# AwsGeek/thinvids

Hardware: AMD Instinct MI355X
Metric: encoded frames/sec (whole node) at fixed PSNR, 1080p & 4K HEVC, 1/2/4/8 MI355X (higher is better)
Workload: dtype uint8 video / int32 integer transforms (bit-exact HEVC)

## Files before the change

### csrc/core/capi.cpp

```cpp
#include <cstring>
#include <exception>
#include <memory>
#include <string>
#include <vector>

#include "tv/av1_enc.h"
#include "tv/container.h"
#include "tv/cpu_encoder.h"
#include "tv/hevc_codec.h"
#include "tv/me_model.h"
#include "tv/sdh.h"
#include "tv/synth.h"
#include "tv/synth_tile.h"
#include "tv/tb_frag.h"

using namespace tv;

namespace {
thread_local std::string g_err;
template <class F> int guard(F&& f) {
  try {
    f();
    return 0;
  } catch (const std::exception& e) {
// ... 110 lines not shown
    uint8_t* P = c == 0 ? y : (c == 1 ? u : v);
    const int pw = c ? cw / 2 : cw, ph = c ? ch / 2 : ch;
    for (int y0 = 0; y0 < ph; y0 += tile_h)
      for (int x0 = 0; x0 < pw; x0 += tile_w)
        synth_tile_fill(ctx, c, x0, y0, tv_min(tile_w, pw - x0), tv_min(tile_h, ph - y0), pw, P);
  }
}

int tv_satd8x8(const int* d, int stride) { return satd8x8(d, stride); }

int tv_sao_picture_cpu(int W, int H, int qp, const uint8_t* sy, const uint8_t* su, const uint8_t* sv,
                       const uint8_t* dy, const uint8_t* du, const uint8_t* dv, uint32_t* params, uint8_t* oy,
                       uint8_t* ou, uint8_t* ov) {
  if (W <= 0 || H <= 0 || W % kCtb || H % kCtb || qp < 0 || qp > 51) {
    g_err = "tv_sao_picture_cpu: bad geometry or QP";
    return -1;
  }
  return guard([&] {
    Picture src, deb;
    src.alloc(W, H);
    deb.alloc(W, H);
    const uint8_t* s[3] = {sy, su, sv};
    const uint8_t* d[3] = {dy, du, dv};
    uint8_t* o[3] = {oy, ou, ov};
    for (int c = 0; c < 3; ++c) {
      const size_t n = (size_t)src.pw(c) * src.ph(c);
      std::memcpy(src.plane(c), s[c], n);
      std::memcpy(deb.plane(c), d[c], n);
    }
    sao_decide_picture(src, deb, qp, params);
    sao_picture(deb, params);
    for (int c = 0; c < 3; ++c) std::memcpy(o[c], deb.plane(c), (size_t)deb.pw(c) * deb.ph(c));
  });
}

void* tv_cpu_encoder_new(int width, int height, int qp, int deblock, int range, int max_merge) {
  SeqConfig cfg;
  cfg.width = width;
  cfg.height = height;
  cfg.qp = qp;
  cfg.set_flags(deblock);
  cfg.max_merge_cand = max_merge;
  cfg.finalize();
  CpuEncoder* e = nullptr;
  guard([&] { e = new CpuEncoder(cfg, range); });
  return e;
}
void* tv_cpu_encoder_new_b(int width, int height, int qp, int deblock, int range, int max_merge, int mgop) {
  SeqConfig cfg;
  cfg.width = width;
  cfg.height = height;
  cfg.qp = qp;
  cfg.set_flags(deblock);
  cfg.max_merge_cand = max_merge;
  cfg.mgop = mgop;
  cfg.finalize();
  CpuEncoder* e = nullptr;
  guard([&] { e = new CpuEncoder(cfg, range); });
  return e;
}
int tv_cpu_encoder_begin_gop(void* e, int nframes, int* disp) {
  return guard([&] {
    auto* enc = static_cast<CpuEncoder*>(e);
    enc->begin_gop(nframes);
    for (size_t k = 0; k < enc->plan().pics.size(); ++k) disp[k] = enc->plan().pics[k].disp;
  });
// ... 248 lines not shown
```

### csrc/gpu/k_frame.hip

```cpp
#include <cstring>

#include "gpu_common.h"
#include "k_encode.h"
#include "tv/synth.h"
#include "tv/synth_tile.h"

namespace tv {
namespace gpu {

constexpr int kSynTW = kSynthTileW, kSynTH = kSynthTileH, kSynRows = kSynTH / 4;
static_assert(kSynTW == 256 && kSynTH % 4 == 0, "a wave of 4-sample items spans the tile; 4 waves share its rows");

struct SynthArgs {
  SynthObject obj[kSynthObjects];
  int32_t t[kMaxBatch];
  int32_t ox[kMaxBatch][kSynthObjects], oy[kMaxBatch][kSynthObjects];
};
static_assert(sizeof(SynthArgs) + sizeof(Geo) + sizeof(FrameSet) + 16 <= 4096, "kernel arguments are limited to 4 KB");

constexpr int kSynSpanX = (kSynTW - 1) * 16, kSynSpanY = (kSynTH - 1) * 16;
constexpr int syn_max(int a, int b) { return a > b ? a : b; }
constexpr int syn_pts(int lp, int s) { return synth_win_max(kSynSpanX << s, lp) * synth_win_max(kSynSpanY << s, lp); }
constexpr int syn_rows(int lp, int s) { return synth_win_max(kSynSpanY << s, lp); }
constexpr int syn_lat_size(bool tex) {
// ... 161 lines not shown
  const int ntx = c ? ncx : nlx, ty = id / ntx, x0 = (id - ty * ntx) * kSynTW, y0 = ty * kSynTH;
  if (c)
    syn_tile<kTex, true>(top, lat, src, g, seed, a, c, x0, y0);
  else
    syn_tile<kTex, false>(top, lat, src, g, seed, a, 0, x0, y0);
}

__global__ void __launch_bounds__(256) k_sse(FrameSet a, FrameSet r, Geo g, unsigned long long* sse) {
  const int c = blockIdx.y, b = blockIdx.z;
  const int pw = c ? g.W / 2 : g.W;
  const int dw = c ? g.dw / 2 : g.dw, dh = c ? g.dh / 2 : g.dh;
  const uint8_t* A = a.plane(c, b, g);
  const uint8_t* R = r.plane(c, b, g);
  const int wq = (dw + 3) >> 2;
  unsigned s = 0;
  for (int i = blockIdx.x * blockDim.x + threadIdx.x; i < wq * dh; i += gridDim.x * blockDim.x) {
    const int y = i / wq, x = (i - y * wq) * 4;
    const uint32_t va = *reinterpret_cast<const uint32_t*>(A + (long)y * pw + x);
    const uint32_t vr = *reinterpret_cast<const uint32_t*>(R + (long)y * pw + x);
#pragma unroll
    for (int k = 0; k < 4; ++k) {
      const int d = (int)((va >> (8 * k)) & 255) - (int)((vr >> (8 * k)) & 255);
      s += (x + k < dw) ? (unsigned)(d * d) : 0u;
    }
  }
  unsigned long long t = s;
  for (int o = 32; o > 0; o >>= 1) t += __shfl_xor(t, o, 64);
  __shared__ unsigned long long part[4];
  if ((threadIdx.x & 63) == 0) part[threadIdx.x >> 6] = t;
  __syncthreads();
  if (threadIdx.x == 0) atomicAdd(sse + b * 3 + c, part[0] + part[1] + part[2] + part[3]);
}

typedef short tv_short2 __attribute__((ext_vector_type(2)));

__device__ constexpr uint32_t pack_taps4(int f, int k0) {
  return (uint32_t)(uint8_t)kLumaFilter[f][k0] | (uint32_t)(uint8_t)kLumaFilter[f][k0 + 1] << 8 |
         (uint32_t)(uint8_t)kLumaFilter[f][k0 + 2] << 16 | (uint32_t)(uint8_t)kLumaFilter[f][k0 + 3] << 24;
}
__device__ constexpr uint32_t pack_taps2(int f, int k0) {
  return (uint32_t)(uint16_t)kLumaFilter[f][k0] | (uint32_t)(uint16_t)kLumaFilter[f][k0 + 1] << 16;
}
__device__ __forceinline__ int dot4(uint32_t a, uint32_t b, int c) {
  return __builtin_amdgcn_sdot4((int)a, (int)b, c, false);
}
__device__ __forceinline__ int dot2(uint32_t a, uint32_t b, int c) {
  return __builtin_amdgcn_sdot2(__builtin_bit_cast(tv_short2, a), __builtin_bit_cast(tv_short2, b), c, false);
}
__device__ __forceinline__ uint32_t pack4_pixels(int v0, int v1, int v2, int v3) {
  return (uint32_t)clip_pixel(v0) | (uint32_t)clip_pixel(v1) << 8 | (uint32_t)clip_pixel(v2) << 16 |
         (uint32_t)clip_pixel(v3) << 24;
}

constexpr int kPhW = 10;
__global__ void __launch_bounds__(256) k_phase_planes(FrameSet ref, uint8_t* phase, Geo g) {
  const int tid = threadIdx.x;
  const int L = xcd_remap(blockIdx.x + gridDim.x * (blockIdx.y + gridDim.y * blockIdx.z),
                          gridDim.x * gridDim.y * gridDim.z);
  const int tpf = gridDim.x * gridDim.y, b = L / tpf, tyi = (L - b * tpf) / gridDim.x;
  const int tx0 = (L - b * tpf - tyi * gridDim.x) * 32 - 8, ty0 = tyi * 32 - 8;
  const uint8_t* R = ref.plane(0, b, g);
  __shared__ uint32_t raw[39][kPhW];
  __shared__ __align__(16) int16_t hf[3][39][32];
  for (int i = tid; i < 39 * kPhW; i += 256) {
    const int rr = i / kPhW, w = i - rr * kPhW;
    const uint8_t* row = R + (long)clip3(0, g.H - 1, ty0 - 3 + rr) * g.W;
    const int x = tx0 - 4 + 4 * w;
    uint32_t v;
    if (x >= 0 && x + 3 < g.W) {
      v = *reinterpret_cast<const uint32_t*>(row + x);
    } else {
      v = 0;
#pragma unroll
      for (int k = 0; k < 4; ++k) v |= (uint32_t)row[clip3(0, g.W - 1, x + k)] << (8 * k);
    }
    raw[rr][w] = v ^ 0x80808080u;
  }
  __syncthreads();
  for (int i = tid; i < 39 * 8; i += 256) {
    const int rr = i >> 3, c4 = i & 7;
    const uint32_t w0 = raw[rr][c4], w1 = raw[rr][c4 + 1], w2 = raw[rr][c4 + 2];
    int out[3][4];
#pragma unroll
    for (int j = 0; j < 4; ++j) {
      const uint32_t lo = j == 3 ? w1 : __builtin_amdgcn_alignbyte(w1, w0, j + 1);
      const uint32_t hi = j == 3 ? w2 : __builtin_amdgcn_alignbyte(w2, w1, j + 1);
#pragma unroll
      for (int f = 1; f < 4; ++f) out[f - 1][j] = dot4(lo, pack_taps4(f, 0), dot4(hi, pack_taps4(f, 4), 8192));
    }
#pragma unroll
    for (int f = 0; f < 3; ++f) {
      uint2 v;
      v.x = (uint32_t)(uint16_t)out[f][0] | (uint32_t)out[f][1] << 16;
      v.y = (uint32_t)(uint16_t)out[f][2] | (uint32_t)out[f][3] << 16;
      *reinterpret_cast<uint2*>(&hf[f][rr][4 * c4]) = v;
    }
  }
  __syncthreads();
  const int r = tid >> 3, c0 = (tid & 7) * 4;
  const int X = tx0 + c0, Y = ty0 + r;
  if (X + 8 >= g.pw16 || Y >= g.H + 8) return;
  uint8_t* base = phase + (long)b * 16 * g.psz + (long)(Y + 8) * g.pw16 + (X + 8);
  auto store = [&](int plane, uint32_t w) { *reinterpret_cast<uint32_t*>(base + (long)plane * g.psz) = w; };
  {
    uint32_t R8[8];
#pragma unroll
    for (int k = 0; k < 8; ++k) R8[k] = raw[r + k][(c0 >> 2) + 1];
    store(0, R8[3] ^ 0x80808080u);
    uint32_t C[2][4];
#pragma unroll
    for (int h = 0; h < 2; ++h) {
      const uint32_t* q = R8 + 4 * h;
      const uint32_t t01l = __builtin_amdgcn_perm(q[1], q[0], 0x05010400u);
      const uint32_t t01h = __builtin_amdgcn_perm(q[1], q[0], 0x07030602u);
      const uint32_t t23l = __builtin_amdgcn_perm(q[3], q[2], 0x05010400u);
      const uint32_t t23h = __builtin_amdgcn_perm(q[3], q[2], 0x07030602u);
      C[h][0] = __builtin_amdgcn_perm(t23l, t01l, 0x05040100u);
      C[h][1] = __builtin_amdgcn_perm(t23l, t01l, 0x07060302u);
      C[h][2] = __builtin_amdgcn_perm(t23h, t01h, 0x05040100u);
      C[h][3] = __builtin_amdgcn_perm(t23h, t01h, 0x07060302u);
    }
#pragma unroll
    for (int fy = 1; fy < 4; ++fy) {
      int v[4];
#pragma unroll
      for (int j = 0; j < 4; ++j)
        v[j] = dot4(C[0][j], pack_taps4(fy, 0), dot4(C[1][j], pack_taps4(fy, 4), 8192 + 32)) >> 6;
      store(4 * fy, pack4_pixels(v[0], v[1], v[2], v[3]));
    }
  }
#pragma unroll
  for (int fx = 1; fx < 4; ++fx) {
    uint2 H8[8];
#pragma unroll
    for (int k = 0; k < 8; ++k) H8[k] = *reinterpret_cast<const uint2*>(&hf[fx - 1][r + k][c0]);
    {
      const int h0 = (int16_t)(H8[3].x & 0xffff), h1 = (int16_t)(H8[3].x >> 16);
      const int h2 = (int16_t)(H8[3].y & 0xffff), h3 = (int16_t)(H8[3].y >> 16);
      store(fx, pack4_pixels((h0 + 32) >> 6, (h1 + 32) >> 6, (h2 + 32) >> 6, (h3 + 32) >> 6));
    }
    uint32_t P[4][4];
#pragma unroll
    for (int m = 0; m < 4; ++m) {
      P[m][0] = __builtin_amdgcn_perm(H8[2 * m + 1].x, H8[2 * m].x, 0x05040100u);
      P[m][1] = __builtin_amdgcn_perm(H8[2 * m + 1].x, H8[2 * m].x, 0x07060302u);
      P[m][2] = __builtin_amdgcn_perm(H8[2 * m + 1].y, H8[2 * m].y, 0x05040100u);
      P[m][3] = __builtin_amdgcn_perm(H8[2 * m + 1].y, H8[2 * m].y, 0x07060302u);
    }
#pragma unroll
    for (int fy = 1; fy < 4; ++fy) {
      int v[4];
#pragma unroll
      for (int j = 0; j < 4; ++j) {
        int a = dot2(P[0][j], pack_taps2(fy, 0), 0);
        a = dot2(P[1][j], pack_taps2(fy, 2), a);
        a = dot2(P[2][j], pack_taps2(fy, 4), a);
        a = dot2(P[3][j], pack_taps2(fy, 6), a);
        v[j] = ((a >> 6) + 32) >> 6;
      }
      store(fx + 4 * fy, pack4_pixels(v[0], v[1], v[2], v[3]));
    }
  }
}

__global__ void __launch_bounds__(256) __attribute__((amdgpu_waves_per_eu(8, 8))) k_deblock(FrameSet rec, DecisionSet dec, Geo g, int horizontal) {
  const int b = blockIdx.y;
  const int qp = dec.qp[b];
  const long ub = b * g.usz;
  const uint8_t* cl = dec.cu_log2 + ub;
  const uint8_t* in = dec.intra + ub;
  const uint8_t* cb = dec.cbf + ub;
  const int16_t* mv = dec.mv + 2 * ub;
  const uint8_t* dir = dec.dir ? dec.dir + ub : nullptr;
  const int16_t* mv1 = dec.mv1 ? dec.mv1 + 2 * ub : nullptr;
  const uint8_t* tu = dec.tu ? dec.tu + ub : nullptr;
  uint8_t* Y = rec.plane(0, b, g);
  uint8_t* U = rec.plane(1, b, g);
  uint8_t* V = rec.plane(2, b, g);
  const int W = g.W, H = g.H, Wc = W / 2;
  const int qpc = chroma_qp(qp, 0);
  const int nl = horizontal ? (H / 8 - 1) * (W / 4) : (W / 8 - 1) * (H / 4);
  const int nc = horizontal ? (H / 16 - 1) * (Wc / 4) : (W / 16 - 1) * (H / 8);
  auto ld = [](const uint8_t* p) { return *reinterpret_cast<const uint32_t*>(p); };
  auto st = [](uint8_t* p, uint32_t v) { *reinterpret_cast<uint32_t*>(p) = v; };
  for (int i = blockIdx.x * blockDim.x + threadIdx.x; i < nl + nc; i += gridDim.x * blockDim.x) {
    if (i < nl) {
      if (!horizontal) {
        const int x = 8 * (1 + i % (W / 8 - 1)), y = 4 * (i / (W / 8 - 1));
        const int bs = deblock_edge_bs(cl, in, cb, mv, g.w8, x - 1, y, x, y, dir, mv1, tu);
        if (bs) {
          uint32_t v[4][2];
#pragma unroll
          for (int k = 0; k < 4; ++k) {
// ... 87 lines not shown
    const int b = (int)(i / f16);
    const long r = i - b * f16;
    const uint4 v = reinterpret_cast<const uint4*>(frames + b * seg_stride)[r];
    uint4* d = r < y16 ? reinterpret_cast<uint4*>(src.y + b * g.ysz) + r
               : r < y16 + c16 ? reinterpret_cast<uint4*>(src.u + b * g.csz) + (r - y16)
                               : reinterpret_cast<uint4*>(src.v + b * g.csz) + (r - y16 - c16);
    *d = v;
  }
}
void launch_gather_frames(const uint8_t* frames, long seg_stride, FrameSet src, const Geo& g, int B, hipStream_t s) {
  const long n = B * (g.ysz + 2 * g.csz) / 16;
  k_gather_frames<<<(unsigned)tv_min(4096L, (n + 255) / 256), 256, 0, s>>>(frames, seg_stride, src, g, B);
}
struct QpArgs {
  int8_t q[64];
};
__global__ void __launch_bounds__(64) k_set_qp(int8_t* dst, QpArgs a, int n) {
  if ((int)threadIdx.x < n) dst[threadIdx.x] = a.q[threadIdx.x];
}
void launch_set_qp(int8_t* dst, const int8_t* host, int n, hipStream_t s) {
  for (int o = 0; o < n; o += 64) {
    QpArgs a;
    const int m = n - o < 64 ? n - o : 64;
    std::memcpy(a.q, host + o, (size_t)m);
    k_set_qp<<<1, 64, 0, s>>>(dst + o, a, m);
  }
}

void launch_sse(FrameSet a, FrameSet r, const Geo& g, unsigned long long* sse, int B, hipStream_t s) {
  dim3 grid((unsigned)tv_min(256, (int)((g.ysz / 4 + 4095) / 4096)), 3, B);
  k_sse<<<grid, 256, 0, s>>>(a, r, g, sse);
}
void launch_phase_planes(FrameSet ref, uint8_t* phase, const Geo& g, int B, hipStream_t s) {
  dim3 grid((g.W + 16 + 31) / 32, (g.H + 16 + 31) / 32, B);
  k_phase_planes<<<grid, 256, 0, s>>>(ref, phase, g);
}
constexpr int kSaoStrip = 4;
constexpr int kSaoRows = 34, kSaoRowsC = 18;
constexpr int kSaoPd = 16 * kSaoStrip + 2, kSaoPdC = 8 * kSaoStrip + 2;
constexpr int kSaoLumaDw = kSaoRows * kSaoPd, kSaoChromaDw = kSaoRowsC * kSaoPdC;
constexpr int kSaoTileDw = kSaoLumaDw + 2 * kSaoChromaDw;
constexpr int kSaoSrcDw = 8 * kSaoStrip + 2, kSaoSrcDwC = 4 * kSaoStrip + 2;
static_assert(kSaoSrcDw <= 64 && kSaoSrcDwC <= 32, "a tile row is staged by one wave (chroma: one half per plane)");
static_assert(8 * (kSaoTileDw * 4 + 64) <= 160 * 1024, "8 workgroups per CU");
typedef short sao_s2 __attribute__((ext_vector_type(2)));
__device__ __forceinline__ sao_s2 sao_pair(uint32_t w) { return __builtin_bit_cast(sao_s2, w); }
typedef unsigned short sao_u2 __attribute__((ext_vector_type(2)));
__device__ __forceinline__ sao_u2 sao_upair(sao_s2 w) { return __builtin_bit_cast(sao_u2, w); }
__device__ __forceinline__ sao_s2 sao_sign2(sao_s2 d) {
  const sao_s2 z = {0, 0};
  const sao_u2 f = {15, 15};
  return (d >> 15) | __builtin_bit_cast(sao_s2, __builtin_bit_cast(sao_u2, z - d) >> f);
}
__device__ __forceinline__ sao_s2 sao_relu2(sao_s2 e) { return e & ~(e >> 15); }
__device__ __forceinline__ sao_s2 sao_pkmax(sao_s2 a, sao_s2 b) {
  uint32_t r;
  asm("v_pk_max_i16 %0, %1, %2" : "=v"(r) : "v"(__builtin_bit_cast(uint32_t, a)), "v"(__builtin_bit_cast(uint32_t, b)));
  return sao_pair(r);
}
__device__ __forceinline__ sao_s2 sao_pkmin(sao_s2 a, sao_s2 b) {
  uint32_t r;
  asm("v_pk_min_i16 %0, %1, %2" : "=v"(r) : "v"(__builtin_bit_cast(uint32_t, a)), "v"(__builtin_bit_cast(uint32_t, b)));
  return sao_pair(r);
}
__device__ __forceinline__ sao_s2 sao_clamp1(sao_s2 d) {
  return sao_pkmin(sao_pkmax(d, sao_s2{-1, -1}), sao_s2{1, 1});
}
// ... 372 lines not shown
```

### csrc/gpu/k_stage.hip

```cpp
#include <hip/hip_runtime.h>

#include <string>

#include "gpu_common.h"
#include "k_encode.h"

namespace tv {
namespace gpu {

__global__ void __launch_bounds__(256) k_pad_plane(const uint8_t* __restrict__ src, int sw, int sh, int sstride, long sfs,
                                                   uint8_t* __restrict__ dst, int pw, int ph, int dstride, long dfs) {
  const int f = blockIdx.z, y = blockIdx.y;
  const int x0 = (blockIdx.x * 256 + threadIdx.x) * 4;
  if (x0 >= pw) return;
  const uint8_t* S = src + f * sfs + (long)tv_min(y, sh - 1) * sstride;
  uint8_t* D = dst + f * dfs + (long)y * dstride;
#pragma unroll
  for (int k = 0; k < 4; ++k)
    if (x0 + k < pw) D[x0 + k] = S[tv_min(x0 + k, sw - 1)];
}

template <typename T>
__global__ void __launch_bounds__(256) k_thumbs8(const T* __restrict__ y, int tw, int stride, long fs, float* out,
                                                 float scale) {
// ... 76 lines not shown
  for (int b = 0; b < B; ++b)
    if (qp[b] < 0 || qp[b] > 51) {
      g_stage_err = "tv_sao_batch: bad QP";
      return -1;
    }
  using namespace tv::gpu;
  hipStream_t st = static_cast<hipStream_t>(stream);
  const Geo g = make_geo(w, h);
  auto set = [&](const uint8_t* p) {
    uint8_t* q = const_cast<uint8_t*>(p);
    return FrameSet{q, q + B * g.ysz, q + B * g.ysz + B * g.csz};
  };
  RcTables t{};
  for (int q = 0; q < 52; ++q) t.sao_lam16[q] = tv::sao_lambda16(q);
  RcTables* rc = nullptr;
  int8_t* dqp = nullptr;
  bool ok = hipMalloc(&rc, sizeof(RcTables)) == hipSuccess && hipMalloc(&dqp, (size_t)B) == hipSuccess &&
            hipMemcpyAsync(rc, &t, sizeof(RcTables), hipMemcpyHostToDevice, st) == hipSuccess &&
            hipMemcpyAsync(dqp, qp, (size_t)B, hipMemcpyHostToDevice, st) == hipSuccess &&
            hipMemsetAsync(sse, 0, (size_t)B * 3 * sizeof(unsigned long long), st) == hipSuccess;
  if (ok) {
    launch_sao(set(src), set(deb), set(out), sao, dqp, rc, g, B, st, sse);
    ok = hipStreamSynchronize(st) == hipSuccess;
  }
  const int rcode = stage_status();
  (void)hipFree(rc);
  (void)hipFree(dqp);
  if (rcode == 0 && !ok) {
    g_stage_err = "tv_sao_batch: device error";
    return -1;
  }
  return rcode;
}
}
```

### thinvids_amd/_abi.py

```python
import ctypes as C

i, l, ll, sz, ull, f32 = C.c_int, C.c_long, C.c_longlong, C.c_size_t, C.c_ulonglong, C.c_float
i32, i64, u32, vp, cstr = C.c_int32, C.c_int64, C.c_uint32, C.c_void_p, C.c_char_p
u8p, i8p, i16p, i32p, u32p = (C.POINTER(t) for t in (C.c_uint8, C.c_int8, C.c_int16, C.c_int32, C.c_uint32))
i64p, u64p, lp, llp, ullp, szp = (C.POINTER(t) for t in (C.c_int64, C.c_uint64, l, ll, ull, sz))
f64p, vpp = C.POINTER(C.c_double), C.POINTER(vp)


class SideTrack(C.Structure):
    _fields_ = [("kind", i32), ("codec", i32), ("timescale", i32), ("channels", i32), ("sample_rate", i32),
                ("bits", i32), ("is_default", i32), ("reserved", i32), ("lang", C.c_char * 4), ("mkv_codec_id", cstr),
                ("priv", vp), ("priv_size", C.c_uint64), ("path", cstr), ("data", vp), ("nsamples", i64),
                ("offsets", vp), ("sizes", vp), ("pts", vp), ("durs", vp)]


CORE = {
    "tv_core_build_hash": (cstr, []),
    "tv_last_error": (cstr, []),
    "tv_core_version": (i, []),
    "tv_bytes_new": (vp, []),
    "tv_bytes_free": (None, [vp]),
    "tv_bytes_size": (sz, [vp]),
    "tv_bytes_data": (vp, [vp]),
    "tv_bytes_clear": (None, [vp]),
    "tv_synth_frame": (None, [u32, i, i, i, u8p, u8p, u8p]),
    "tv_synth_frame_tiled": (None, [u32, i, i, i, i, i, u8p, u8p, u8p]),
    "tv_satd8x8": (i, [i32p, i]),
    "tv_sao_picture_cpu": (i, [i, i, i] + [u8p] * 6 + [u32p] + [u8p] * 3),
    "tv_cpu_encoder_new": (vp, [i] * 6),
    "tv_cpu_encoder_new_b": (vp, [i] * 7),
    "tv_cpu_encoder_new_crf": (vp, [i] * 7),
    "tv_cpu_encoder_free": (None, [vp]),
    "tv_cpu_encoder_begin_gop": (i, [vp, i, i32p]),
    "tv_gop_plan": (i, [i, i] + [i32p] * 6),
    "tv_cpu_encoder_encode": (i, [vp, u8p, u8p, u8p, i, i, i, i, vp]),
    "tv_cpu_encoder_encode_qp": (i, [vp, u8p, u8p, u8p, i, i, i, i, i, vp]),
    "tv_cpu_encoder_recon": (None, [vp, u8p, u8p, u8p]),
    "tv_cpu_encoder_decisions": (None, [vp, u8p, u8p, u8p, i16p, u8p]),
    "tv_cpu_encoder_levels": (None, [vp, i16p, i16p, i16p]),
    "tv_reconstruct_frame": (i, [i] * 4 + [u8p] * 9 + [i16p, u8p, i16p, i16p, i16p, u8p, u8p, u8p]),
    "tv_write_frame": (i, [i] * 7 + [u8p, u8p, u8p, i16p, u8p, i16p, i16p, i16p, vp]),
    "tv_mv_rate": (None, [i32p, i32p, i, i32p, i32p]),
    "tv_av1_mv_comp_bits": (None, [i32p, i, i32p]),
    "tv_tb_frag_expand": (i, [i, i32p]),
    "tv_quant_levels": (None, [i32p, i, i, i, i32p, i32p]),
    "tv_sdh_deltas": (None, [i32p, i, i, i, i, i32p, i32p]),
    "tv_hevc_spec_table": (i, [cstr, i32p, i]),
    "tv_decoder_new": (vp, []),
    "tv_decoder_free": (None, [vp]),
    "tv_decoder_decode": (i, [vp, u8p, sz]),
    "tv_decoder_decode_range": (i, [vp, u8p, sz, i, i]),
    "tv_decoder_info": (None, [vp] + [i32p] * 5),
    "tv_decoder_frame": (i, [vp, i, i, u8p, u8p, u8p]),
    "tv_hevc_scale_mv": (None, [i, i, i, i, i32p]),
    "tv_hevc_display_offsets": (i, [u8p, sz, i32p, i]),
    "tv_hevc_probe": (i, [u8p, sz] + [i32p] * 4),
    "tv_mux_mp4": (i, [u8p, sz, i, i, i, i, vp]),
    "tv_mux_mp4_file": (i, [vpp, szp, i, i, i, i, i, cstr, ullp]),
    "tv_mux_file": (i, [vpp, szp, i, i, i, i, i, C.POINTER(SideTrack), i, i, cstr, ullp]),
    "tv_side_track_size": (sz, []),
    "tv_demux_mp4": (i, [u8p, sz] + [i32p] * 5 + [vp]),
# ... 37 lines not shown
    "tv_mpeg2_raps": (i, [u8p, sz, i64p, i64p, i32p, i32p, i]),
    "tv_mpeg2_decode": (i, [u8p, sz, i64, i64, i32, i32, i32, u8p, i32p, i64p]),
    "tv_mpeg2_table": (i, [i, i32p, i32p, i32p, i]),
    "tv_mpeg2_stat_name": (cstr, [i]),
    "tv_mpeg2_num_stats": (i, []),
}

GPU = {
    "tv_gpu_build_hash": (cstr, []),
    "tv_gpu_last_error": (cstr, []),
    "tv_gpu_device_count": (i, []),
    "tv_engine_new_b": (vp, [i] * 7 + [u32, i, i, i, i, i]),
    "tv_engine_free": (None, [vp]),
    "tv_engine_encode_synth": (i, [vp, i32p, i, i, vp]),
    "tv_engine_encode_host": (i, [vp, u8p, i, i, vp]),
    "tv_engine_encode_device": (i, [vp, vp, i, i, vp]),
    "tv_engine_segment_size": (sz, [vp, i]),
    "tv_engine_segment_copy": (None, [vp, i, u8p]),
    "tv_engine_sse": (None, [vp, i, f64p]),
    "tv_engine_timing": (None, [vp] + [f64p] * 4),
    "tv_engine_entropy_stats": (None, [vp, i32p, llp, i32p]),
    "tv_engine_entropy_host_pictures": (ll, [vp]),
    "tv_engine_entropy_lane_pictures": (ll, [vp, i]),
    "tv_engine_estimate": (i, [i] * 6 + [ullp, ullp]),
    "tv_engine_footprint": (None, [vp, ullp, ullp]),
    "tv_engine_last_recon": (i, [vp, i, u8p, u8p, u8p]),
    "tv_ingest_last_error": (cstr, []),
    "tv_ingest_h2d": (i, [cstr, ll, ll, vp, vp, ll, i, vp, f64p]),
    "tv_stage_last_error": (cstr, []),
    "tv_thumbs8_batch": (i, [vp, i, i, i, i, l, i, vp, vp]),
    "tv_pad_batch": (i, [vp, i, i, i, l, vp, i, i, i, l, i, vp]),
    "tv_synth_batch": (i, [vp, i, i, i, i32p, u32, vp]),
    "tv_sao_batch": (i, [vp, vp, vp, vp, vp, i, i, i, i8p, vp]),
    "tv_ops_last_error": (cstr, []),
    "tv_resize_plane": (i, [vp, i, i, i, vp, i, i, i, vp, vp, i, vp, vp, i, vp, vp]),
    "tv_resize_batch": (i, [vp, i, i, i, l, vp, i, i, i, l, i, i, i, vp, vp, i, vp, vp, i, vp, i, i, i, vp]),
    "tv_rgb_to_i420": (i, [vp, i, i, i, vp, vp, vp, i, vp]),
    "tv_p010_to_i420": (i, [vp, vp, i, i, vp, vp, vp, vp]),
    "tv_tonemap_pq": (i, [vp, vp, i, i, vp, vp, vp, f32, f32, vp]),
    "tv_tonemap_pq_batch": (i, [vp, vp, i, i, i, vp, f32, f32, vp]),
    "tv_synth_p010": (i, [vp, vp, i, i, i, i, u32, vp]),
    "tv_overlay_mask": (i, [vp, i, i, i, vp, i, i, i, i, vp]),
    "tv_bwdif_segment": (i, [vp, vp, l, i, i, lp, i32p, i32p, i, vp]),
    "tv_bwdif_plane": (i, [vp, vp, vp, vp, i, i, i, vp]),
    "tv_ssim_plane": (i, [vp, vp, i, i, i, i, vp, vp]),
    "tv_av1_gpu_last_error": (cstr, []),
    "tv_gpu_cdef_dirs": (i, [vp, i, i, i, vp, vp, vp]),
    "tv_gpu_cdef_search": (i, [vp, vp, i, i, i, i, vp, vp, i, i, i, vp, vp, ull, i]),
    "tv_gpu_cdef_apply": (i, [vp, i, i, i, i, vp, vp, i, i, i, vp, vp, vp]),
    "tv_gpu_sgr_select": (i, [vp, vp, vp, i, i, i, i, vp, vp, vp, vp]),
    "tv_gpu_wiener_apply": (i, [vp, i, i, i, vp, vp, vp]),
    "tv_gpu_wiener_stats": (i, [vp, vp, i, i, i, i, vp, vp, vp]),
    "tv_gpu_sgr_stats": (i, [vp, vp, i, i, i, i, vp, vp]),
    "tv_gpu_sgr_apply": (i, [vp, i, i, i, vp, vp, vp]),
    "tv_gpu_av1_deblock_step": (i, [vp, vp, i, i, i, i, vp, i, i, vp]),
    "tv_av1_txfm_last_error": (cstr, []),
    "tv_gpu_av1_txfm": (i, [vp, vp, i, i, i, vp, vp, vp]),
    "tv_av1e_last_error": (cstr, []),
    "tv_av1e_inter": (i, [vp] * 18 + [i, i, i, vp, vp]),
    "tv_av1e_iblocks": (i, [vp] * 16 + [i, i, i, vp, i, vp]),
    "tv_av1e_intra": (i, [vp] * 11 + [i, i, i, vp, i, vp]),
    "tv_av1e_cdef_skip": (i, [vp, vp, i, i, i, vp]),
    "tv_av1e_merge": (i, [vp, vp, i, i, i, vp]),
    "tv_av1e_tb_len": (i, [vp, vp, l, i, i, i, i, vp, vp]),
    "tv_av1e_tb_pack": (i, [vp, vp, vp, l, i, i, i, i, vp, vp]),
    "tv_av1e_lfinfo": (i, [vp, i, i, i, vp, vp, vp, vp, vp]),
# ... 4 lines not shown
```

### thinvids_amd/models/hevc.py

```python
from __future__ import annotations

import ctypes as C
import threading
from dataclasses import dataclass

import numpy as np

from .._native import Bytes, check, core_lib, ok, ptr

Frame = tuple


def coded_size(width: int, height: int, ctb: int = 32) -> tuple[int, int]:
    return (width + ctb - 1) // ctb * ctb, (height + ctb - 1) // ctb * ctb


def synth_frame(seed: int, t: int, width: int, height: int) -> Frame:
    y = np.empty((height, width), np.uint8)
    u = np.empty((height // 2, width // 2), np.uint8)
    v = np.empty_like(u)
    core_lib().tv_synth_frame(seed & 0xFFFFFFFF, t, width, height, ptr(y), ptr(u), ptr(v))
    return y, u, v


def sao_picture_cpu(src: Frame, deb: Frame, qp: int) -> tuple[np.ndarray, Frame]:
    h, w = deb[0].shape
    src = [np.ascontiguousarray(p, np.uint8) for p in src]
    deb = [np.ascontiguousarray(p, np.uint8) for p in deb]
    params = np.empty((h // 32, w // 32, 3), np.uint32)
    out = [np.empty_like(p) for p in deb]
    check(core_lib().tv_sao_picture_cpu(w, h, qp, *[ptr(p) for p in src], *[ptr(p) for p in deb], ptr(params),
                                        *[ptr(p) for p in out]))
    return params, tuple(out)


def psnr(a: np.ndarray, b: np.ndarray) -> float:
    mse = np.mean((a.astype(np.float64) - b.astype(np.float64)) ** 2)
    return float("inf") if mse == 0 else 10.0 * np.log10(255.0 ** 2 / mse)


def psnr_yuv(ref: Frame, dec: Frame) -> dict:
    py, pu, pv = (psnr(r, d) for r, d in zip(ref, dec))
    return {"y": py, "u": pu, "v": pv, "yuv": (6 * py + pu + pv) / 8}


FLAG_DEBLOCK = 1
FLAG_SAO = 2
FLAG_WPP = 4
FLAG_NO_RQT = 8
FLAG_NO_PINTRA = 16
FLAG_HOST_ENTROPY = 32
FLAG_CASCADE = 64
FLAG_NO_RDOQ = 128
FLAG_SUBPEL_SATD = 256
FLAG_SIGN_HIDING = 512


def codec_flags(deblock: bool = True, sao: bool = False, wpp: bool = True, rqt: bool = True, pintra: bool = True,
                cascade: bool = False, rdoq: bool = True, subpel_satd: bool = False, sign_hiding: bool = False) -> int:
    on = {FLAG_DEBLOCK: deblock, FLAG_SAO: sao, FLAG_WPP: wpp, FLAG_NO_RQT: not rqt, FLAG_NO_PINTRA: not pintra,
          FLAG_CASCADE: cascade, FLAG_NO_RDOQ: not rdoq, FLAG_SUBPEL_SATD: subpel_satd, FLAG_SIGN_HIDING: sign_hiding}
    return sum(bit for bit, v in on.items() if v)


IPPP_CASCADE_IDR = -5
IPPP_CASCADE_P = (1, 0, 1, -1, 1, 0, 1, -3)
# ... 272 lines not shown
```

### thinvids_amd/ops/stage.py

```python
from __future__ import annotations

import ctypes as C
import threading
from dataclasses import dataclass, field

import numpy as np

from .._native import gpu_lib, ok, stream
from ..models.hevc import coded_size


_lib = gpu_lib


def _ok(rc: int, which: str = "stage") -> None:
    ok(rc, gpu_lib(), f"tv_{which}_last_error")


@dataclass
class DevFrames:
    buf: object
    n: int
    w: int
    h: int
# ... 77 lines not shown
    _ok(_lib().tv_synth_batch(buf.data_ptr(), w, h, n, ts, seed & 0xFFFFFFFF, stream(device)))
    planes = [(0, w, h, cw, ysz), (n * ysz, w // 2, h // 2, cw // 2, csz),
              (n * ysz + n * csz, w // 2, h // 2, cw // 2, csz)]
    return DevFrames(buf, n, w, h, planes, 8)


def sao_pictures(src, deb, w: int, h: int, qps, device):
    import torch

    B = len(deb)
    cw, ch = coded_size(w, h)

    def batched(pics):
        flat = np.concatenate([np.ascontiguousarray(p[c], np.uint8).reshape(-1) for c in range(3) for p in pics])
        assert flat.size == B * cw * ch * 3 // 2, "pictures must have the coded size"
        return torch.from_numpy(flat).to(device)

    ds, dd = batched(src), batched(deb)
    out = torch.empty_like(dd)
    nctb = (cw // 32) * (ch // 32)
    prm = torch.empty(B * nctb * 3, dtype=torch.int32, device=device)
    sse = torch.empty(B * 3, dtype=torch.int64, device=device)
    q = (C.c_int8 * B)(*[int(x) for x in qps])
    torch.cuda.current_stream(device).synchronize()
    _ok(_lib().tv_sao_batch(ds.data_ptr(), dd.data_ptr(), out.data_ptr(), prm.data_ptr(), sse.data_ptr(), w, h, B, q,
                            stream(device)))
    o = out.cpu().numpy()
    ysz, csz = cw * ch, cw * ch // 4
    pics = [(o[b * ysz:(b + 1) * ysz].reshape(ch, cw),
             o[B * ysz + b * csz:B * ysz + (b + 1) * csz].reshape(ch // 2, cw // 2),
             o[B * (ysz + csz) + b * csz:B * (ysz + csz) + (b + 1) * csz].reshape(ch // 2, cw // 2)) for b in range(B)]
    return (prm.cpu().numpy().view(np.uint32).reshape(B, ch // 32, cw // 32, 3), pics,
            sse.cpu().numpy().view(np.uint64).reshape(B, 3))


def tone_map(src: DevFrames, src_peak: float = 1000.0, dst_peak: float = 100.0) -> DevFrames:
    import torch

    if src.bits != 10:
        return src
    n, w, h = src.n, src.w, src.h
    dev = src.buf.device
    (yo, _, _, ys, yfs), (uo, _, _, us, ufs), (vo, _, _, vs, vfs) = src.planes
    flat = src.buf.reshape(-1)

    def plane(off, pw, ph, stride, fs):
        return torch.as_strided(flat, (n, ph, pw), (fs, stride, 1), off).to(torch.int32)

    y16 = (plane(yo, w, h, ys, yfs) << 6).to(torch.int16).contiguous()
    u = plane(uo, w // 2, h // 2, us, ufs) << 6
    v = plane(vo, w // 2, h // 2, vs, vfs) << 6
    uv16 = torch.stack([u, v], -1).reshape(n, h // 2, w).to(torch.int16).contiguous()
    fsz = w * h * 3 // 2
    out = torch.empty((n, fsz), dtype=torch.uint8, device=dev)
    _ok(_lib().tv_tonemap_pq_batch(y16.data_ptr(), uv16.data_ptr(), w, h, n, out.data_ptr(), src_peak, dst_peak,
                                   stream(dev)), "ops")
    res = DevFrames(out, n, w, h, flat_layout(w, h), 8)
    res.keep = [y16, uv16]
    return res


def staging_planes(w: int, h: int, coded: tuple | None = None) -> tuple[int, list]:
    cw, ch = coded or coded_size(w, h)
    ysz, csz = cw * ch, (cw // 2) * (ch // 2)
    return ysz + 2 * csz, [(0, w, h, cw, cw, ch), (ysz, w // 2, h // 2, cw // 2, cw // 2, ch // 2),
                           (ysz + csz, w // 2, h // 2, cw // 2, cw // 2, ch // 2)]
# ... 88 lines not shown
```

Before: 13010.

## Compute luma quarter-pel phase planes with MFMA int8 matrix ops

Rewrites k_phase_planes so the 8-tap horizontal and vertical luma interpolation runs as banded-matrix products on MFMA i32_16x16x32_i8 instead of sdot4/sdot2 dot products. Tiles widen to 64 columns, and the intermediate horizontal result is stored transposed in LDS, split into signed high and low bytes for the second MFMA pass. It also adds a CPU reference function and a batch test entry point for checking bit-exactness. The gain depends on MFMA throughput beating the extra shuffling and LDS transposes, and the byte-split arithmetic risks rounding errors.

```diff
diff --git a/csrc/core/capi.cpp b/csrc/core/capi.cpp
--- a/csrc/core/capi.cpp
+++ b/csrc/core/capi.cpp
@@ -166,6 +166,19 @@
     sao_picture(deb, params);
     for (int c = 0; c < 3; ++c) std::memcpy(o[c], deb.plane(c), (size_t)deb.pw(c) * deb.ph(c));
   });
+}
+
+int tv_phase_planes_cpu(int W, int H, const uint8_t* ref, uint8_t* out) {
+  if (W <= 0 || H <= 0 || W % kCtb || H % kCtb) {
+    g_err = "tv_phase_planes_cpu: bad geometry";
+    return -1;
+  }
+  const int pw = W + 16, ph = H + 16;
+  for (int p = 0; p < 16; ++p)
+    for (int y = 0; y < ph; ++y)
+      for (int x = 0; x < pw; ++x)
+        out[((size_t)p * ph + y) * pw + x] = (uint8_t)mc_luma_sample(ref, W, W, H, x - 8, y - 8, p & 3, p >> 2);
+  return 0;
 }
 
 void* tv_cpu_encoder_new(int width, int height, int qp, int deblock, int range, int max_merge) {
diff --git a/csrc/gpu/k_frame.hip b/csrc/gpu/k_frame.hip
--- a/csrc/gpu/k_frame.hip
+++ b/csrc/gpu/k_frame.hip
@@ -217,39 +217,40 @@
   if (threadIdx.x == 0) atomicAdd(sse + b * 3 + c, part[0] + part[1] + part[2] + part[3]);
 }
 
-typedef short tv_short2 __attribute__((ext_vector_type(2)));
-
-__device__ constexpr uint32_t pack_taps4(int f, int k0) {
-  return (uint32_t)(uint8_t)kLumaFilter[f][k0] | (uint32_t)(uint8_t)kLumaFilter[f][k0 + 1] << 8 |
-         (uint32_t)(uint8_t)kLumaFilter[f][k0 + 2] << 16 | (uint32_t)(uint8_t)kLumaFilter[f][k0 + 3] << 24;
-}
-__device__ constexpr uint32_t pack_taps2(int f, int k0) {
-  return (uint32_t)(uint16_t)kLumaFilter[f][k0] | (uint32_t)(uint16_t)kLumaFilter[f][k0 + 1] << 16;
-}
-__device__ __forceinline__ int dot4(uint32_t a, uint32_t b, int c) {
-  return __builtin_amdgcn_sdot4((int)a, (int)b, c, false);
-}
-__device__ __forceinline__ int dot2(uint32_t a, uint32_t b, int c) {
-  return __builtin_amdgcn_sdot2(__builtin_bit_cast(tv_short2, a), __builtin_bit_cast(tv_short2, b), c, false);
-}
-__device__ __forceinline__ uint32_t pack4_pixels(int v0, int v1, int v2, int v3) {
-  return (uint32_t)clip_pixel(v0) | (uint32_t)clip_pixel(v1) << 8 | (uint32_t)clip_pixel(v2) << 16 |
-         (uint32_t)clip_pixel(v3) << 24;
-}
-
-constexpr int kPhW = 10;
-__global__ void __launch_bounds__(256) k_phase_planes(FrameSet ref, uint8_t* phase, Geo g) {
-  const int tid = threadIdx.x;
+typedef int tv_int4 __attribute__((ext_vector_type(4)));
+
+constexpr int kPhRows = 40;
+constexpr int kPhPitch = 72;
+constexpr int kPhImg = 64 * kPhRows + 8;
+
+__device__ constexpr uint64_t pack_taps8(int f) {
+  uint64_t v = 0;
+  for (int k = 0; k < 8; ++k) v |= (uint64_t)(uint8_t)kLumaFilter[f][k] << (8 * k);
+  return v;
+}
+__device__ __forceinline__ long tap_band(uint64_t taps, int n, int q) {
+  const int s = 8 * (n + 1) - 64 * q;
+  const uint64_t v = (s >= 64 || s <= -64) ? 0 : (s >= 0 ? taps << s : taps >> -s);
+  return (long)v;
+}
+typedef unsigned short tv_ushort2 __attribute__((ext_vector_type(2)));
+__device__ __forceinline__ uint32_t pack4_pixels_shr12(int v0, int v1, int v2, int v3) {
+  const tv_ushort2 p = {__builtin_amdgcn_ashr_pk_u8_i32(v0, v1, 12), __builtin_amdgcn_ashr_pk_u8_i32(v2, v3, 12)};
+  return __builtin_bit_cast(uint32_t, p);
+}
+
+__global__ void __launch_bounds__(256) __attribute__((amdgpu_waves_per_eu(4))) k_phase_planes(FrameSet ref, uint8_t* phase, Geo g) {
+  const int tid = threadIdx.x, wv = tid >> 6, n = tid & 15, q = (tid >> 4) & 3;
   const int L = xcd_remap(blockIdx.x + gridDim.x * (blockIdx.y + gridDim.y * blockIdx.z),
                           gridDim.x * gridDim.y * gridDim.z);
   const int tpf = gridDim.x * gridDim.y, b = L / tpf, tyi = (L - b * tpf) / gridDim.x;
-  const int tx0 = (L - b * tpf - tyi * gridDim.x) * 32 - 8, ty0 = tyi * 32 - 8;
+  const int tx0 = (L - b * tpf - tyi * gridDim.x) * 64 - 8, ty0 = tyi * 32 - 8;
   const uint8_t* R = ref.plane(0, b, g);
-  __shared__ uint32_t raw[39][kPhW];
-  __shared__ __align__(16) int16_t hf[3][39][32];
-  for (int i = tid; i < 39 * kPhW; i += 256) {
-    const int rr = i / kPhW, w = i - rr * kPhW;
-    const uint8_t* row = R + (long)clip3(0, g.H - 1, ty0 - 3 + rr) * g.W;
+  __shared__ __align__(16) uint8_t raw[kPhRows * kPhPitch + 8];
+  __shared__ __align__(16) uint8_t img[4][2][kPhImg];
+  for (int i = tid; i < kPhRows * (kPhPitch / 4); i += 256) {
+    const int rr = i / (kPhPitch / 4), w = i - rr * (kPhPitch / 4);
+    const uint8_t* row = R + (long)clip3(0, g.H - 1, ty0 - 4 + rr) * g.W;
     const int x = tx0 - 4 + 4 * w;
     uint32_t v;
     if (x >= 0 && x + 3 < g.W) {
@@ -259,91 +260,56 @@
 #pragma unroll
       for (int k = 0; k < 4; ++k) v |= (uint32_t)row[clip3(0, g.W - 1, x + k)] << (8 * k);
     }
-    raw[rr][w] = v ^ 0x80808080u;
-  }
+    reinterpret_cast<uint32_t*>(raw)[i] = v ^ 0x80808080u;
+  }
+  long band[4];
+#pragma unroll
+  for (int f = 0; f < 4; ++f) band[f] = tap_band(pack_taps8(f), n, q);
   __syncthreads();
-  for (int i = tid; i < 39 * 8; i += 256) {
-    const int rr = i >> 3, c4 = i & 7;
-    const uint32_t w0 = raw[rr][c4], w1 = raw[rr][c4 + 1], w2 = raw[rr][c4 + 2];
-    int out[3][4];
-#pragma unroll
-    for (int j = 0; j < 4; ++j) {
-      const uint32_t lo = j == 3 ? w1 : __builtin_amdgcn_alignbyte(w1, w0, j + 1);
-      const uint32_t hi = j == 3 ? w2 : __builtin_amdgcn_alignbyte(w2, w1, j + 1);
-#pragma unroll
-      for (int f = 1; f < 4; ++f) out[f - 1][j] = dot4(lo, pack_taps4(f, 0), dot4(hi, pack_taps4(f, 4), 8192));
-    }
-#pragma unroll
-    for (int f = 0; f < 3; ++f) {
-      uint2 v;
-      v.x = (uint32_t)(uint16_t)out[f][0] | (uint32_t)out[f][1] << 16;
-      v.y = (uint32_t)(uint16_t)out[f][2] | (uint32_t)out[f][3] << 16;
-      *reinterpret_cast<uint2*>(&hf[f][rr][4 * c4]) = v;
+#pragma unroll
+  for (int m = 0; m < 3; ++m) {
+    const int rr = tv_min(16 * m + n, kPhRows - 1);
+    const long a = *reinterpret_cast<const long*>(raw + rr * kPhPitch + 16 * wv + 8 * q);
+    const bool keep = 16 * m + 4 * q < kPhRows;
+#pragma unroll
+    for (int f = 0; f < 4; ++f) {
+      const tv_int4 h = __builtin_amdgcn_mfma_i32_16x16x32_i8(a, band[f], tv_int4{8192, 8192, 8192, 8192}, 0, 0, 0);
+      const uint32_t p01 = __builtin_amdgcn_perm((uint32_t)h[1], (uint32_t)h[0], 0x05010400u);
+      const uint32_t p23 = __builtin_amdgcn_perm((uint32_t)h[3], (uint32_t)h[2], 0x05010400u);
+      if (keep) {
+        uint8_t* at = &img[f][0][(16 * wv + n) * kPhRows + 16 * m + 4 * q];
+        *reinterpret_cast<uint32_t*>(at) = __builtin_amdgcn_perm(p23, p01, 0x07060302u);
+        *reinterpret_cast<uint32_t*>(at + kPhImg) = __builtin_amdgcn_perm(p23, p01, 0x05040100u) ^ 0x80808080u;
+      }
     }
   }
   __syncthreads();
-  const int r = tid >> 3, c0 = (tid & 7) * 4;
-  const int X = tx0 + c0, Y = ty0 + r;
-  if (X + 8 >= g.pw16 || Y >= g.H + 8) return;
-  uint8_t* base = phase + (long)b * 16 * g.psz + (long)(Y + 8) * g.pw16 + (X + 8);
-  auto store = [&](int plane, uint32_t w) { *reinterpret_cast<uint32_t*>(base + (long)plane * g.psz) = w; };
-  {
-    uint32_t R8[8];
-#pragma unroll
-    for (int k = 0; k < 8; ++k) R8[k] = raw[r + k][(c0 >> 2) + 1];
-    store(0, R8[3] ^ 0x80808080u);
-    uint32_t C[2][4];
-#pragma unroll
-    for (int h = 0; h < 2; ++h) {
-      const uint32_t* q = R8 + 4 * h;
-      const uint32_t t01l = __builtin_amdgcn_perm(q[1], q[0], 0x05010400u);
-      const uint32_t t01h = __builtin_amdgcn_perm(q[1], q[0], 0x07030602u);
-      const uint32_t t23l = __builtin_amdgcn_perm(q[3], q[2], 0x05010400u);
-      const uint32_t t23h = __builtin_amdgcn_perm(q[3], q[2], 0x07030602u);
-      C[h][0] = __builtin_amdgcn_perm(t23l, t01l, 0x05040100u);
-      C[h][1] = __builtin_amdgcn_perm(t23l, t01l, 0x07060302u);
-      C[h][2] = __builtin_amdgcn_perm(t23h, t01h, 0x05040100u);
-      C[h][3] = __builtin_amdgcn_perm(t23h, t01h, 0x07060302u);
-    }
-#pragma unroll
-    for (int fy = 1; fy < 4; ++fy) {
-      int v[4];
-#pragma unroll
-      for (int j = 0; j < 4; ++j)
-        v[j] = dot4(C[0][j], pack_taps4(fy, 0), dot4(C[1][j], pack_taps4(fy, 4), 8192 + 32)) >> 6;
-      store(4 * fy, pack4_pixels(v[0], v[1], v[2], v[3]));
-    }
-  }
-#pragma unroll
-  for (int fx = 1; fx < 4; ++fx) {
-    uint2 H8[8];
-#pragma unroll
-    for (int k = 0; k < 8; ++k) H8[k] = *reinterpret_cast<const uint2*>(&hf[fx - 1][r + k][c0]);
-    {
-      const int h0 = (int16_t)(H8[3].x & 0xffff), h1 = (int16_t)(H8[3].x >> 16);
-      const int h2 = (int16_t)(H8[3].y & 0xffff), h3 = (int16_t)(H8[3].y >> 16);
-      store(fx, pack4_pixels((h0 + 32) >> 6, (h1 + 32) >> 6, (h2 + 32) >> 6, (h3 + 32) >> 6));
-    }
-    uint32_t P[4][4];
-#pragma unroll
-    for (int m = 0; m < 4; ++m) {
-      P[m][0] = __builtin_amdgcn_perm(H8[2 * m + 1].x, H8[2 * m].x, 0x05040100u);
-      P[m][1] = __builtin_amdgcn_perm(H8[2 * m + 1].x, H8[2 * m].x, 0x07060302u);
-      P[m][2] = __builtin_amdgcn_perm(H8[2 * m + 1].y, H8[2 * m].y, 0x05040100u);
-      P[m][3] = __builtin_amdgcn_perm(H8[2 * m + 1].y, H8[2 * m].y, 0x07060302u);
-    }
-#pragma unroll
-    for (int fy = 1; fy < 4; ++fy) {
-      int v[4];
-#pragma unroll
-      for (int j = 0; j < 4; ++j) {
-        int a = dot2(P[0][j], pack_taps2(fy, 0), 0);
-        a = dot2(P[1][j], pack_taps2(fy, 2), a);
-        a = dot2(P[2][j], pack_taps2(fy, 4), a);
-        a = dot2(P[3][j], pack_taps2(fy, 6), a);
-        v[j] = ((a >> 6) + 32) >> 6;
-      }
-      store(fx + 4 * fy, pack4_pixels(v[0], v[1], v[2], v[3]));
+  const int fx = wv, X = tx0 + 16 * q;
+  const bool in_x = X + 8 < g.pw16;
+#pragma unroll
+  for (int rb = 0; rb < 2; ++rb) {
+    long ah[4], al[4];
+#pragma unroll
+    for (int t = 0; t < 4; ++t) {
+      const uint8_t* at = &img[fx][0][(16 * (n >> 2) + 4 * t + (n & 3)) * kPhRows + 16 * rb + 8 * q];
+      ah[t] = *reinterpret_cast<const long*>(at);
+      al[t] = *reinterpret_cast<const long*>(at + kPhImg);
+    }
+    const int Y = ty0 + 16 * rb + n;
+    const bool in = in_x && Y < g.H + 8;
+    uint8_t* base = phase + (long)b * 16 * g.psz + (long)(Y + 8) * g.pw16 + (X + 8);
+#pragma unroll
+    for (int fy = 0; fy < 4; ++fy) {
+      uint4 o;
+      uint32_t* ow = reinterpret_cast<uint32_t*>(&o);
+#pragma unroll
+      for (int t = 0; t < 4; ++t) {
+        const tv_int4 hi = __builtin_amdgcn_mfma_i32_16x16x32_i8(ah[t], band[fy], tv_int4{0, 0, 0, 0}, 0, 0, 0);
+        const tv_int4 lo =
+            __builtin_amdgcn_mfma_i32_16x16x32_i8(al[t], band[fy], tv_int4{10240, 10240, 10240, 10240}, 0, 0, 0);
+        ow[t] = pack4_pixels_shr12(hi[0] * 256 + lo[0], hi[1] * 256 + lo[1], hi[2] * 256 + lo[2], hi[3] * 256 + lo[3]);
+      }
+      if (in) *reinterpret_cast<uint4*>(base + (long)(fx + 4 * fy) * g.psz) = o;
     }
   }
 }
@@ -497,7 +463,7 @@
   k_sse<<<grid, 256, 0, s>>>(a, r, g, sse);
 }
 void launch_phase_planes(FrameSet ref, uint8_t* phase, const Geo& g, int B, hipStream_t s) {
-  dim3 grid((g.W + 16 + 31) / 32, (g.H + 16 + 31) / 32, B);
+  dim3 grid((g.W + 16 + 63) / 64, (g.H + 16 + 31) / 32, B);
   k_phase_planes<<<grid, 256, 0, s>>>(ref, phase, g);
 }
 constexpr int kSaoStrip = 4;
diff --git a/csrc/gpu/k_stage.hip b/csrc/gpu/k_stage.hip
--- a/csrc/gpu/k_stage.hip
+++ b/csrc/gpu/k_stage.hip
@@ -132,4 +132,22 @@
   }
   return rcode;
 }
+
+int tv_phase_planes_batch(const uint8_t* luma, uint8_t* phase, int w, int h, int B, void* stream) {
+  if (w < 2 || h < 2 || (w & 1) || (h & 1) || B <= 0 || B > tv::gpu::kMaxBatch) {
+    g_stage_err = "tv_phase_planes_batch: bad geometry";
+    return -1;
+  }
+  using namespace tv::gpu;
+  hipStream_t st = static_cast<hipStream_t>(stream);
+  const Geo g = make_geo(w, h);
+  launch_phase_planes(FrameSet{const_cast<uint8_t*>(luma), nullptr, nullptr}, phase, g, B, st);
+  const bool ok = hipStreamSynchronize(st) == hipSuccess;
+  const int rcode = stage_status();
+  if (rcode == 0 && !ok) {
+    g_stage_err = "tv_phase_planes_batch: device error";
+    return -1;
+  }
+  return rcode;
 }
+}
diff --git a/thinvids_amd/_abi.py b/thinvids_amd/_abi.py
--- a/thinvids_amd/_abi.py
+++ b/thinvids_amd/_abi.py
@@ -27,6 +27,7 @@
     "tv_synth_frame_tiled": (None, [u32, i, i, i, i, i, u8p, u8p, u8p]),
     "tv_satd8x8": (i, [i32p, i]),
     "tv_sao_picture_cpu": (i, [i, i, i] + [u8p] * 6 + [u32p] + [u8p] * 3),
+    "tv_phase_planes_cpu": (i, [i, i, u8p, u8p]),
     "tv_cpu_encoder_new": (vp, [i] * 6),
     "tv_cpu_encoder_new_b": (vp, [i] * 7),
     "tv_cpu_encoder_new_crf": (vp, [i] * 7),
@@ -130,6 +131,7 @@
     "tv_pad_batch": (i, [vp, i, i, i, l, vp, i, i, i, l, i, vp]),
     "tv_synth_batch": (i, [vp, i, i, i, i32p, u32, vp]),
     "tv_sao_batch": (i, [vp, vp, vp, vp, vp, i, i, i, i8p, vp]),
+    "tv_phase_planes_batch": (i, [vp, vp, i, i, i, vp]),
     "tv_ops_last_error": (cstr, []),
     "tv_resize_plane": (i, [vp, i, i, i, vp, i, i, i, vp, vp, i, vp, vp, i, vp, vp]),
     "tv_resize_batch": (i, [vp, i, i, i, l, vp, i, i, i, l, i, i, i, vp, vp, i, vp, vp, i, vp, i, i, i, vp]),
diff --git a/thinvids_amd/models/hevc.py b/thinvids_amd/models/hevc.py
--- a/thinvids_amd/models/hevc.py
+++ b/thinvids_amd/models/hevc.py
@@ -32,6 +32,14 @@
     check(core_lib().tv_sao_picture_cpu(w, h, qp, *[ptr(p) for p in src], *[ptr(p) for p in deb], ptr(params),
                                         *[ptr(p) for p in out]))
     return params, tuple(out)
+
+
+def phase_planes_cpu(luma: np.ndarray) -> np.ndarray:
+    luma = np.ascontiguousarray(luma, np.uint8)
+    h, w = luma.shape
+    out = np.empty((16, h + 16, w + 16), np.uint8)
+    check(core_lib().tv_phase_planes_cpu(w, h, ptr(luma), ptr(out)))
+    return out
 
 
 def psnr(a: np.ndarray, b: np.ndarray) -> float:
diff --git a/thinvids_amd/ops/stage.py b/thinvids_amd/ops/stage.py
--- a/thinvids_amd/ops/stage.py
+++ b/thinvids_amd/ops/stage.py
@@ -133,6 +133,24 @@
              o[B * (ysz + csz) + b * csz:B * (ysz + csz) + (b + 1) * csz].reshape(ch // 2, cw // 2)) for b in range(B)]
     return (prm.cpu().numpy().view(np.uint32).reshape(B, ch // 32, cw // 32, 3), pics,
             sse.cpu().numpy().view(np.uint64).reshape(B, 3))
+
+
+def phase_planes(lumas, w: int, h: int, device):
+    import torch
+
+    B = len(lumas)
+    cw, ch = coded_size(w, h)
+    flat = np.concatenate([np.ascontiguousarray(p, np.uint8).reshape(-1) for p in lumas])
+    assert flat.size == B * cw * ch, "pictures must have the coded size"
+    src = torch.from_numpy(flat).to(device)
+    n, guard = B * 16 * (cw + 16) * (ch + 16), 4096
+    buf = torch.full((n + 2 * guard,), 0xA5, dtype=torch.uint8, device=device)
+    torch.cuda.current_stream(device).synchronize()
+    _ok(_lib().tv_phase_planes_batch(src.data_ptr(), buf.data_ptr() + guard, w, h, B, stream(device)))
+    o = buf.cpu().numpy()
+    if not ((o[:guard] == 0xA5).all() and (o[guard + n:] == 0xA5).all()):
+        raise RuntimeError("tv_phase_planes_batch wrote outside the phase buffer")
+    return o[guard:guard + n].reshape(B, 16, ch + 16, cw + 16)
 
 
 def tone_map(src: DevFrames, src_peak: float = 1000.0, dst_peak: float = 100.0) -> DevFrames:
```

Measured after the change: 13330, median of 3. About the same (+2.4%).
